# InfiniTensor/InfiniTensor

Hardware: AMD Instinct MI355X
Metric: bf16 MatMul 4096x4096x4096 throughput (GEMM TFLOP/s, % dense MFMA peak) (higher is better)
Workload: dtype bf16; 1 GPU; BASELINE configs[1]: one bf16 MatMul M=N=K=4096 per GPU, NN layout, fp32 accumulate, via infini_rocm_matmul; kernel_variant=heuristic, kernel_variant_launched=wave128, device=AMD Radeon Graphics, arch=gfx950:sramecc+:xnack-, compute_units=256, clock_mhz=2400, parallelism=1 independent replicas (column-sharded GEMM has no collective)

## Files before the change

infinitensor_amd/csrc/gemm128w.hip:

```cpp
#include "gemm256_common.h"
#include "diag.h"

namespace irocm {
namespace g128w {

using g256::mn_f;
using g256::sfor;

constexpr int kStage = 32768, kOper = 16384;
constexpr int kLds = 4 * kStage;
constexpr int kGroupM = 4;

struct WArgs {
    GemmArgs g;
    int total_tiles;
    int dbg;
    unsigned long long *stamps;
};
#ifdef IROCM_DIAG
constexpr bool kDiag = true;
#else
constexpr bool kDiag = false;
#endif
constexpr int kStamps = 8;

template <bool KMAJOR> struct Frags;
template <> struct Frags<true> {
    s16x8_t v[3][8];
    unsigned base[2];
    __device__ __forceinline__ void init(unsigned lds_oper, int half, int l15, int g4) {
        const int slot = (l15 & 1) | (((l15 >> 3) & 1) << 1) | (((l15 >> 1) & 3) << 2);
        base[0] = lds_oper + (unsigned)(half * 8192 + slot * 64 + ((g4 ^ (slot >> 2)) & 3) * 16);
        base[1] = base[0] + 2u * kStage;
    }
    template <int SET, int F, int STAGE, int DST = F> __device__ __forceinline__ void read0() {
        asm volatile("ds_read_b128 %0, %1 offset:%2" : "=v"(v[SET][DST]) : "v"(base[STAGE >> 1]), "i"(F * 1024 + (STAGE & 1) * kStage));
    }
    template <int SET, int F, int STAGE, int DST = F> __device__ __forceinline__ void read1() {}
    template <int SET, int F> __device__ __forceinline__ s16x8_t get() const { return v[SET][F]; }
};
template <> struct Frags<false> {
    s16x4_t lo[3][8], hi[3][8];
    unsigned addr[8];
    __device__ __forceinline__ void init(unsigned lds_oper, int half, int l15, int g4) {
        const int mnf = ((l15 >> 2) & 3) | ((g4 & 1) << 2);
        const unsigned mn_lane = (unsigned)((g4 * 8 + (l15 >> 2)) * 512 + (l15 & 1) * 8);
#pragma unroll
        for (int f = 0; f < 8; ++f) {
            const int c16 = ((l15 >> 1) & 1) | (((half * 8 + f) ^ mnf) << 1);
            addr[f] = lds_oper + mn_lane + (unsigned)c16 * 16u;
        }
    }
    template <int SET, int F, int STAGE, int DST = F> __device__ __forceinline__ void read0() {
        const unsigned a = STAGE >= 2 ? addr[F] + 2u * kStage : addr[F];
        asm volatile("ds_read_b64_tr_b16 %0, %1 offset:%2" : "=v"(lo[SET][DST]) : "v"(a), "i"((STAGE & 1) * kStage));
    }
    template <int SET, int F, int STAGE, int DST = F> __device__ __forceinline__ void read1() {
        const unsigned a = STAGE >= 2 ? addr[F] + 2u * kStage : addr[F];
        asm volatile("ds_read_b64_tr_b16 %0, %1 offset:%2" : "=v"(hi[SET][DST]) : "v"(a), "i"((STAGE & 1) * kStage + 2048));
    }
    template <int SET, int F> __device__ __forceinline__ s16x8_t get() const {
        return s16x8_t{lo[SET][F][0], lo[SET][F][1], lo[SET][F][2], lo[SET][F][3], hi[SET][F][0], hi[SET][F][1], hi[SET][F][2], hi[SET][F][3]};
    }
};

template <bool KMAJOR> __device__ __forceinline__ void piece_offs(unsigned (&off)[4], long ld, int w, int lane) {
#pragma unroll
    for (int i = 0; i < 4; ++i) {
        const int piece = w * 4 + i;
        if constexpr (KMAJOR) {
            const int slot = lane >> 2;
            const int r = piece * 16 + ((slot & 1) | (((slot >> 2) & 3) << 1) | (((slot >> 1) & 1) << 3));
            const int c_log = (lane & 3) ^ ((slot >> 2) & 3);
            off[i] = (unsigned)(((long)r * ld + c_log * 8) * 2);
        } else {
            const int kr = piece * 2 + (lane >> 5);
            const int c_log = (lane & 31) ^ (mn_f(kr) << 1);
            off[i] = (unsigned)(((long)kr * ld + c_log * 8) * 2);
        }
    }
}

struct PieceSel {
    int oper, idx, stage, imm;
};
template <bool AKM, bool BKM> constexpr int step_pieces(int S) { return (AKM ? ((S & 1) ? 8 : 0) : 4) + (BKM ? ((S & 1) ? 8 : 0) : 4); }
template <bool AKM, bool BKM> constexpr PieceSel piece_sel(int S, int q) {
    const int na = AKM ? ((S & 1) ? 8 : 0) : 4;
    const int oper = q < na ? 0 : 1, r = q < na ? q : q - na;
    const bool km = oper == 0 ? AKM : BKM;
    if (!km)
        return {oper, r, (S + 3) & 3, 0};
    return {oper, r >> 1, (r & 1) ? (S & 3) : ((S + 3) & 3), (r & 1) * 64};
}
constexpr int slot_piece(int n, int I, int slot) {
    if (n == 0)
        return -1;
    if (n <= 8) {
        const int stride = 8 / n;
        return (slot == 0 && I % stride == 0) ? I / stride : -1;
    }
    return slot == 0 ? I : (8 + I < n ? 8 + I : -1);
}

template <typename Tr> __device__ __forceinline__ unsigned cvt_pk_a(float lo, float hi) {
    unsigned r;
    if constexpr (Tr::kDType == INFINI_DT_BF16) asm volatile("v_cvt_pk_bf16_f32 %0, %1, %2" : "=v"(r) : "v"(lo), "v"(hi));
    else asm volatile("v_cvt_pk_f16_f32 %0, %1, %2" : "=v"(r) : "v"(lo), "v"(hi));
    return r;
}
#ifdef IROCM_W128_C_WB
#define W128_ST_MOD ""
#else
#define W128_ST_MOD " sc0 sc1"
#endif
struct EpiUnit {
    int kind, jp, t;
};
constexpr int kEpiUnits = 60;
constexpr EpiUnit epi_unit(int e) {
    const int kind[12] = {0, 0, 1, 0, 2, 1, 0, 2, 1, 2, 1, 2};
    const int jp[12] = {0, 1, 0, 2, 0, 1, 3, 1, 2, 2, 3, 3};
    const int size[12] = {12, 12, 2, 12, 1, 2, 12, 1, 2, 1, 2, 1};
    int s = 0;
    for (int i = 0; i < 12; ++i) {
        if (e < s + size[i])
            return {kind[i], jp[i], e - s};
        s += size[i];
    }
    return {-1, 0, 0};
}

template <typename Tr, bool FIRST> __device__ __forceinline__ void mfma_a(f32x4 &acc, s16x8_t x, s16x8_t y) {
    if constexpr (Tr::kDType == INFINI_DT_BF16) {
        if constexpr (FIRST) asm volatile("v_mfma_f32_16x16x32_bf16 %0, %1, %2, 0" : "=a"(acc) : "v"(x), "v"(y));
        else asm volatile("v_mfma_f32_16x16x32_bf16 %0, %1, %2, %0" : "+a"(acc) : "v"(x), "v"(y));
    } else {
        if constexpr (FIRST) asm volatile("v_mfma_f32_16x16x32_f16 %0, %1, %2, 0" : "=a"(acc) : "v"(x), "v"(y));
        else asm volatile("v_mfma_f32_16x16x32_f16 %0, %1, %2, %0" : "+a"(acc) : "v"(x), "v"(y));
    }
}

template <typename Tr, bool AKM, bool BKM>
__global__ __launch_bounds__(256, 1) void gemm128w_kernel(WArgs pw) {
    extern __shared__ __attribute__((aligned(1024))) char smem[];
    const GemmArgs &p = pw.g;
    unsigned long long tc0 = 0, tr0 = 0;
    if constexpr (kDiag) {
        tc0 = __builtin_amdgcn_s_memtime();
        tr0 = __builtin_amdgcn_s_memrealtime();
    }
    const int t = threadIdx.x, lane = t & 63, l15 = lane & 15, g4 = lane >> 4;
    int w;
    asm volatile("v_readfirstlane_b32 %0, %1" : "=s"(w) : "v"(t >> 6));
    const int wr = w >> 1, wc = w & 1;
    const unsigned lds0 = (unsigned)(unsigned long)IROCM_LDS_PTR(smem);
    unsigned lds0s;
    asm volatile("v_readfirstlane_b32 %0, %1" : "=s"(lds0s) : "v"(lds0));

    const long lda = AKM ? p.a_rs : p.a_cs, ldb = BKM ? p.b_cs : p.b_rs;
    unsigned a_kstep = (unsigned)(AKM ? 64 : 64 * lda), b_kstep = (unsigned)(BKM ? 64 : 64 * ldb);
    const long a_tile = AKM ? 512 * lda : 512, b_tile = BKM ? 512 * ldb : 512;
    unsigned a_off[4], b_off[4];
    piece_offs<AKM>(a_off, lda, w, lane);
    piece_offs<BKM>(b_off, ldb, w, lane);
    if (pw.dbg & 2) {
        a_kstep = b_kstep = 0;
#pragma unroll
        for (int i = 0; i < 4; ++i) a_off[i] = b_off[i] = (unsigned)lane * 16u;
    }
    const int ksteps = p.k >> 5, nkb = ksteps >> 2;
    const unsigned a_span = a_kstep * (unsigned)ksteps, b_span = b_kstep * (unsigned)ksteps;

    const unsigned grid = gridDim.x, wg = xcd_remap(blockIdx.x, grid);
    const unsigned per_batch = (unsigned)(p.tiles_m * p.tiles_n);
    auto decode = [&](unsigned tile, const char *&ab, const char *&bb, long &c_elem) {
        const unsigned ib = tile / per_batch, r = tile - ib * per_batch;
        const unsigned gspan = (unsigned)(kGroupM * p.tiles_n), grp = r / gspan, i = r - grp * gspan;
        const unsigned first_m = grp * kGroupM;
        const unsigned gsz = (unsigned)p.tiles_m - first_m < (unsigned)kGroupM ? (unsigned)p.tiles_m - first_m : (unsigned)kGroupM;
        const unsigned tn = i / gsz, tm = first_m + (i - tn * gsz);
        ab = (const char *)p.a + ((long)ib * p.a_bs) * 2 + (long)tm * a_tile;
        bb = (const char *)p.b + ((long)ib * p.b_bs) * 2 + (long)tn * b_tile;
        c_elem = (long)ib * p.c_bs + (long)tm * 256 * p.n + (long)tn * 256;
    };
    auto uniform = [](const char *q) {
        const unsigned long v = (unsigned long)q;
        const unsigned lo = __builtin_amdgcn_readfirstlane((unsigned)v), hi = __builtin_amdgcn_readfirstlane((unsigned)(v >> 32));
        return (const char *)(((unsigned long)hi << 32) | lo);
    };

    unsigned tile = wg;
    const char *pa, *pb;
    long c_elem;
    decode(tile, pa, pb, c_elem);
    pa = uniform(pa);
    pb = uniform(pb);

    unsigned m0w = lds0s + (unsigned)w * 4096u;
    auto load_piece = [&](auto operc, auto idxc, auto immc) __attribute__((always_inline)) {
        constexpr int OP = decltype(operc)::value, IDX = decltype(idxc)::value, IMM = decltype(immc)::value;
        const unsigned off = OP == 0 ? a_off[IDX] : b_off[IDX];
        const char *base = OP == 0 ? pa : pb;
        asm volatile("global_load_lds_dwordx4 %0, %1 offset:%2" ::"v"(off), "s"(base), "i"(IMM) : "memory");
    };
    auto set_m0 = [&m0w](auto stc, auto operc, auto idxc, auto immc) __attribute__((always_inline)) {
        constexpr int ST = decltype(stc)::value, OP = decltype(operc)::value, IDX = decltype(idxc)::value, IMM = decltype(immc)::value;
        const unsigned m0base = m0w;
        asm volatile("s_add_u32 m0, %0, %1" ::"s"(m0base), "i"(ST * kStage + OP * kOper + IDX * 1024 - IMM) : "memory", "scc");
    };
    auto pin = [&]() __attribute__((always_inline)) { asm volatile("" : "+s"(pa), "+s"(pb)); };
    auto request = [&](auto stc, auto operc) __attribute__((always_inline)) {
        constexpr int ST = decltype(stc)::value, OP = decltype(operc)::value;
        constexpr bool KM = OP == 0 ? AKM : BKM;
        sfor<4>([&](auto idxc) {
            set_m0(stc, operc, idxc, std::integral_constant<int, 0>{});
            asm volatile("s_nop 0" ::: "memory");
            load_piece(operc, idxc, std::integral_constant<int, 0>{});
            if constexpr (KM) {
                set_m0(std::integral_constant<int, ST + 1>{}, operc, idxc, std::integral_constant<int, 64>{});
                asm volatile("s_nop 0" ::: "memory");
                load_piece(operc, idxc, std::integral_constant<int, 64>{});
            }
        });
    };
    auto advance = [&](auto operc, unsigned by) __attribute__((always_inline)) {
#pragma unroll
        for (int i = 0; i < 4; ++i) {
            if constexpr (decltype(operc)::value == 0) a_off[i] += by;
            else b_off[i] += by;
        }
    };
    constexpr std::integral_constant<int, 0> kA{};
    constexpr std::integral_constant<int, 1> kB{};

    Frags<AKM> fa;
    Frags<BKM> fb;
    fa.init(lds0, wr, l15, g4);
    fb.init(lds0 + kOper, wc, l15, g4);
    f32x4 acc[8][8];

    constexpr int nKM = (AKM ? 1 : 0) + (BKM ? 1 : 0), nMN = 2 - nKM;
    pin();
    asm volatile("s_nop 4" ::: "memory");
    if constexpr (AKM) request(std::integral_constant<int, 0>{}, kA);
    if constexpr (BKM) request(std::integral_constant<int, 0>{}, kB);
    if constexpr (!AKM) request(std::integral_constant<int, 0>{}, kA);
    if constexpr (!BKM) request(std::integral_constant<int, 0>{}, kB);
    if constexpr (AKM) advance(kA, 128);
    else advance(kA, a_kstep);
    if constexpr (BKM) advance(kB, 128);
    else advance(kB, b_kstep);
    if constexpr (!AKM) request(std::integral_constant<int, 1>{}, kA);
    if constexpr (!BKM) request(std::integral_constant<int, 1>{}, kB);
    if constexpr (!AKM) advance(kA, a_kstep);
    if constexpr (!BKM) advance(kB, b_kstep);
    if constexpr (AKM) request(std::integral_constant<int, 2>{}, kA);
    if constexpr (BKM) request(std::integral_constant<int, 2>{}, kB);
    if constexpr (!AKM) request(std::integral_constant<int, 2>{}, kA);
    if constexpr (!BKM) request(std::integral_constant<int, 2>{}, kB);
    if constexpr (AKM) advance(kA, 128);
    else advance(kA, a_kstep);
    if constexpr (BKM) advance(kB, 128);
    else advance(kB, b_kstep);
    constexpr int kG1 = 4 * nMN, kG2 = 8 * nKM + 4 * nMN;
    asm volatile("s_waitcnt vmcnt(%0)" ::"n"(kG1 + kG2) : "memory");
    __builtin_amdgcn_s_barrier();
    sfor<8>([&](auto fc) {
        constexpr int F = decltype(fc)::value;
        fa.template read0<0, F, 0>();
        fa.template read1<0, F, 0>();
        fb.template read0<0, F, 0>();
        fb.template read1<0, F, 0>();
    });
    asm volatile("s_waitcnt vmcnt(%0) lgkmcnt(0)" ::"n"(kG2) : "memory");
    __builtin_amdgcn_s_barrier();

    const char *na = pa, *nb = pb;
    auto step = [&](auto sc, auto firstc, bool last_block) __attribute__((always_inline)) {
        constexpr int S = decltype(sc)::value;
        constexpr bool FIRST = decltype(firstc)::value;
        constexpr int CUR = S & 1, NXT = CUR ^ 1, RS = (S + 1) & 3, NP = step_pieces<AKM, BKM>(S);
        sfor<8>([&](auto ic) {
            constexpr int I = decltype(ic)::value;
            sfor<8>([&](auto jc) {
                constexpr int J = decltype(jc)::value;
                mfma_a<Tr, FIRST>(acc[I][J], fb.template get<CUR, J>(), fa.template get<CUR, I>());
                if constexpr (J == 0) fa.template read0<NXT, I, RS>();
                if constexpr (J == 1) fa.template read1<NXT, I, RS>();
                if constexpr (J == 2) fb.template read0<NXT, I, RS>();
                if constexpr (J == 3) fb.template read1<NXT, I, RS>();
                if constexpr (J >= 4) {
                    constexpr int Q = slot_piece(NP, I, (J - 4) >> 1);
                    if constexpr (Q >= 0) {
                        constexpr PieceSel ps = piece_sel<AKM, BKM>(S, Q);
                        if constexpr ((J & 1) == 0)
                            set_m0(std::integral_constant<int, ps.stage>{}, std::integral_constant<int, ps.oper>{}, std::integral_constant<int, ps.idx>{},
                                   std::integral_constant<int, ps.imm>{});
                        else
                            load_piece(std::integral_constant<int, ps.oper>{}, std::integral_constant<int, ps.idx>{}, std::integral_constant<int, ps.imm>{});
                    }
                }
            });
        });
        if (S == 0 && last_block) {
            pa = na;
            pb = nb;
            pin();
            advance(kA, AKM ? 0u - a_span : a_kstep - a_span);
            advance(kB, BKM ? 0u - b_span : b_kstep - b_span);
        } else {
            if constexpr (!AKM) advance(kA, a_kstep);
            else if constexpr (S & 1) advance(kA, 128);
            if constexpr (!BKM) advance(kB, b_kstep);
            else if constexpr (S & 1) advance(kB, 128);
        }
        asm volatile("s_waitcnt vmcnt(%0) lgkmcnt(0)" ::"n"(NP) : "memory");
        __builtin_amdgcn_s_barrier();
    };
    constexpr std::integral_constant<int, 0> k0{};
    constexpr std::integral_constant<int, 1> k1{};
    constexpr std::integral_constant<int, 2> k2{};
    constexpr std::integral_constant<int, 3> k3{};
    auto block = [&](auto firstc, bool last_block) __attribute__((always_inline)) {
        step(k0, firstc, last_block);
        step(k1, std::false_type{}, last_block);
        step(k2, std::false_type{}, last_block);
        step(k3, std::false_type{}, last_block);
    };
    unsigned long long tc_first = 0, tr_first = 0, tc_mfma = 0, tr_mfma = 0, tc_store = 0;
    if constexpr (kDiag) {
        tc_first = __builtin_amdgcn_s_memtime();
        tr_first = __builtin_amdgcn_s_memrealtime();
    }
    const unsigned total = (unsigned)pw.total_tiles;
    const long ldc2 = (long)p.n * 2;
    auto final_block = [&]() __attribute__((always_inline)) {
        const int ln = (int)__builtin_amdgcn_mbcnt_hi(~0u, __builtin_amdgcn_mbcnt_lo(~0u, 0u));
        const unsigned c_lane = (unsigned)(((long)(ln & 15) * p.n + ((ln >> 4) & 1) * 16 + (ln >> 5) * 8) * 2);
        char *cw = (char *)p.c + (c_elem + (long)wr * 128 * p.n + wc * 128) * 2;
        cw = (char *)uniform(cw);
        unsigned pu[8], pv[8];
        float t0 = 0.f, t1 = 0.f;
        sfor<8>([&](auto ic) {
            constexpr int I = decltype(ic)::value;
            constexpr int SA = (I & 1) * 2, SN = ((I + 1) & 1) * 2;
            char *cb = cw + (long)(I > 0 ? I - 1 : 0) * 16 * ldc2;
            asm volatile("" : "+s"(cb));
            if constexpr (I > 0) asm volatile("s_waitcnt lgkmcnt(0)" ::: "memory");
            sfor<24>([&](auto mc) {
                constexpr int M = decltype(mc)::value, KS = M >> 3, J = M & 7;
                if constexpr (I == 0 && M == 8) {
                    asm volatile("s_waitcnt vmcnt(0) lgkmcnt(0)" ::: "memory");
                    __builtin_amdgcn_s_barrier();
                }
                if constexpr (I == 0 && M == 16) asm volatile("s_waitcnt lgkmcnt(0)" ::: "memory");
                if constexpr (KS == 0) mfma_a<Tr, false>(acc[I][J], fb.template get<1, J>(), fa.template get<1, I>());
                if constexpr (KS == 1) mfma_a<Tr, false>(acc[I][J], fb.template get<0, J>(), fa.template get<0, SA>());
                if constexpr (KS == 2) mfma_a<Tr, false>(acc[I][J], fb.template get<2, J>(), fa.template get<0, SA + 1>());
                if constexpr (I == 0 && KS == 0) {
                    fb.template read0<0, J, 2>();
                    fb.template read1<0, J, 2>();
                    if constexpr (J == 0) {
                        fa.template read0<0, 0, 2, 0>();
                        fa.template read1<0, 0, 2, 0>();
                    }
                }
                if constexpr (I == 0 && KS == 1) {
                    fb.template read0<2, J, 3>();
                    fb.template read1<2, J, 3>();
                    if constexpr (J == 0) {
                        fa.template read0<0, 0, 3, 1>();
                        fa.template read1<0, 0, 3, 1>();
                    }
                }
                if constexpr (I < 7 && M == 16) {
                    fa.template read0<0, I + 1, 2, SN>();
                    fa.template read1<0, I + 1, 2, SN>();
                }
                if constexpr (I < 7 && M == 17) {
                    fa.template read0<0, I + 1, 3, SN + 1>();
                    fa.template read1<0, I + 1, 3, SN + 1>();
                }
                if constexpr (I > 0) {
                    constexpr int R = I - 1, E0 = M * kEpiUnits / 24, E1 = (M + 1) * kEpiUnits / 24;
                    sfor<E1 - E0>([&](auto uc) {
                        constexpr EpiUnit un = epi_unit(E0 + decltype(uc)::value);
                        if constexpr (un.kind == 0) {
                            constexpr int Q = 2 * un.jp + un.t / 6, H = (un.t % 6) / 3, RR = un.t % 3;
                            if constexpr (RR < 2) {
                                const float src = acc[R][Q][2 * H + RR];
                                float dst;
                                asm volatile("v_accvgpr_read_b32 %0, %1" : "=v"(dst) : "a"(src));
                                if constexpr (RR == 0) t0 = dst;
                                else t1 = dst;
                            } else if constexpr (un.t < 6) {
                                pu[2 * un.jp + H] = cvt_pk_a<Tr>(t0, t1);
                            } else {
                                pv[2 * un.jp + H] = cvt_pk_a<Tr>(t0, t1);
                            }
                        } else if constexpr (un.kind == 1) {
                            unsigned x = pu[2 * un.jp + un.t], y = pv[2 * un.jp + un.t];
                            asm volatile("v_permlane16_swap_b32 %0, %1" : "+v"(x), "+v"(y));
                            pu[2 * un.jp + un.t] = x;
                            pv[2 * un.jp + un.t] = y;
                        } else {
                            const u32x4_t d = u32x4_t{pu[2 * un.jp], pu[2 * un.jp + 1], pv[2 * un.jp], pv[2 * un.jp + 1]};
                            const unsigned cl = c_lane;
                            char *cbs = cb;
                            asm volatile("global_store_dwordx4 %0, %1, %2 offset:%3" W128_ST_MOD ::"v"(cl), "v"(d), "s"(cbs), "i"(un.jp * 64) : "memory");
                        }
                    });
                }
            });
        });
    };
    auto epilogue = [&](auto firstrowc) __attribute__((always_inline)) {
        constexpr int FIRSTROW = decltype(firstrowc)::value;
        if constexpr (kDiag) {
            tc_mfma = __builtin_amdgcn_s_memtime();
            tr_mfma = __builtin_amdgcn_s_memrealtime();
        }
        asm volatile("s_nop 15\n\ts_nop 15" ::: "memory");
        const int ln = (int)__builtin_amdgcn_mbcnt_hi(~0u, __builtin_amdgcn_mbcnt_lo(~0u, 0u));
        const unsigned c_lane = (unsigned)(((long)(ln & 15) * p.n + ((ln >> 4) & 1) * 16 + (ln >> 5) * 8) * 2);
        char *cw = (char *)p.c + (c_elem + (long)wr * 128 * p.n + wc * 128) * 2;
        cw = (char *)uniform(cw);
        if (!(pw.dbg & 1))
        sfor<8>([&](auto ic) {
            constexpr int I = decltype(ic)::value;
            if constexpr (I < FIRSTROW) return;
            char *cb = cw + (long)I * 16 * ldc2;
            asm volatile("s_nop 4" : "+s"(cb));
            unsigned u[8], v[8];
#pragma unroll
            for (int jp = 0; jp < 4; ++jp) {
                const f32x4 x = acc[I][2 * jp], y = acc[I][2 * jp + 1];
                u[2 * jp] = Tr::pack2(x[0], x[1]);
                u[2 * jp + 1] = Tr::pack2(x[2], x[3]);
                v[2 * jp] = Tr::pack2(y[0], y[1]);
                v[2 * jp + 1] = Tr::pack2(y[2], y[3]);
            }
            asm volatile("s_nop 1\n\t"
                         "v_permlane16_swap_b32 %0, %8\n\tv_permlane16_swap_b32 %1, %9\n\tv_permlane16_swap_b32 %2, %10\n\t"
                         "v_permlane16_swap_b32 %3, %11\n\tv_permlane16_swap_b32 %4, %12\n\tv_permlane16_swap_b32 %5, %13\n\t"
                         "v_permlane16_swap_b32 %6, %14\n\tv_permlane16_swap_b32 %7, %15"
                         : "+v"(u[0]), "+v"(u[1]), "+v"(u[2]), "+v"(u[3]), "+v"(u[4]), "+v"(u[5]), "+v"(u[6]), "+v"(u[7]), "+v"(v[0]), "+v"(v[1]),
                           "+v"(v[2]), "+v"(v[3]), "+v"(v[4]), "+v"(v[5]), "+v"(v[6]), "+v"(v[7]));
            const u32x4_t d0 = u32x4_t{u[0], u[1], v[0], v[1]}, d1 = u32x4_t{u[2], u[3], v[2], v[3]};
            const u32x4_t d2 = u32x4_t{u[4], u[5], v[4], v[5]}, d3 = u32x4_t{u[6], u[7], v[6], v[7]};
            const unsigned cl = c_lane;
            asm volatile("global_store_dwordx4 %0, %1, %5" W128_ST_MOD "\n\tglobal_store_dwordx4 %0, %2, %5 offset:64" W128_ST_MOD "\n\t"
                         "global_store_dwordx4 %0, %3, %5 offset:128" W128_ST_MOD "\n\tglobal_store_dwordx4 %0, %4, %5 offset:192" W128_ST_MOD "\n\ts_nop 1" ::"v"(cl),
                         "v"(d0), "v"(d1), "v"(d2), "v"(d3), "s"(cb)
                         : "memory");
        });
        if constexpr (kDiag) tc_store = __builtin_amdgcn_s_memtime();
    };
    for (; tile + grid < total; tile += grid) {
        {
            long dummy;
            decode(tile + grid, na, nb, dummy);
            na = uniform(na);
            nb = uniform(nb);
        }
        block(std::true_type{}, nkb == 1);
        for (int kb = 1; kb < nkb; ++kb) block(std::false_type{}, kb == nkb - 1);
        epilogue(k0);
        const char *ta, *tb;
        decode(tile + grid, ta, tb, c_elem);
    }
    if (nkb == 1) {
        step(k0, std::true_type{}, false);
        final_block();
        epilogue(std::integral_constant<int, 7>{});
    } else {
        block(std::true_type{}, false);
        for (int kb = 1; kb < nkb - 1; ++kb) block(std::false_type{}, false);
        step(k0, std::false_type{}, false);
        final_block();
        epilogue(std::integral_constant<int, 7>{});
    }
    asm volatile("s_waitcnt vmcnt(0)" ::: "memory");
    if constexpr (kDiag) {
        const bool lane0 = w == 0 && __builtin_amdgcn_mbcnt_hi(~0u, __builtin_amdgcn_mbcnt_lo(~0u, 0u)) == 0;
        if ((pw.dbg & 16) && lane0) {
            unsigned long long *d = pw.stamps + (size_t)blockIdx.x * kStamps;
            d[0] = tc0, d[1] = tc_first, d[2] = tc_mfma, d[3] = tc_store, d[4] = __builtin_amdgcn_s_memtime();
            d[5] = tr0, d[6] = tr_mfma, d[7] = __builtin_amdgcn_s_memrealtime();
        }
        if ((pw.dbg & 8) && blockIdx.x == 0 && lane0) {
            unsigned long long *d = (unsigned long long *)p.c;
            d[0] = __builtin_amdgcn_s_memtime() - tc_first;
            d[1] = __builtin_amdgcn_s_memrealtime() - tr_first;
        }
    }
}

template <typename Tr> static int launch_t(infiniRocmRuntime_t rt, GemmArgs p, bool akm, bool bkm) {
    WArgs w;
    p.tiles_m = p.m / 256;
    p.tiles_n = p.n / 256;
    w.g = p;
    w.total_tiles = p.tiles_m * p.tiles_n * p.batch;
    const char *dbg = diag_getenv("IROCM_W128_DBG");
    w.dbg = dbg ? atoi(dbg) : 0;
    w.stamps = nullptr;
    const unsigned grid = (unsigned)(w.total_tiles < rt->num_cu ? w.total_tiles : rt->num_cu);
    if (w.dbg & 16) {
        void *ws = nullptr;
        if (int st = infini_rocm_workspace(rt, (size_t)grid * kStamps * sizeof(unsigned long long), &ws))
            return st;
        w.stamps = (unsigned long long *)ws;
    }
    return with_layout(akm, bkm, [&](auto ak, auto bk) -> int {
        auto kern = gemm128w_kernel<Tr, decltype(ak)::value, decltype(bk)::value>;
        IROCM_LDS_ATTR(kern, kLds, rt);
        hipLaunchKernelGGL(kern, dim3(grid), dim3(256), kLds, rt->stream, w);
        IROCM_LAUNCH_CHECK("gemm128w");
        return INFINI_ROCM_OK;
    });
}

int launch_gemm128w(infiniRocmRuntime_t rt, int dtype, const GemmArgs &p, bool akm, bool bkm) {
    if (!wave128_supported(gemm_problem(p, dtype, akm, bkm)))
        IROCM_FAIL(INFINI_ROCM_UNSUPPORTED, "gemm128w: this problem is outside the four-wave kernel's contract (gemm_route.h)");
    return dtype == INFINI_DT_BF16 ? launch_t<Bf16Traits>(rt, p, akm, bkm) : launch_t<F16Traits>(rt, p, akm, bkm);
}

}
}
```

Before: 1550 TFLOP/s.

## Precompute tile-decode constants on host and use magic-number division in kernel

Moves per-launch derived values (strides in bytes, tile counts, k-steps, spans, XCD remap quotient/remainder) into a flattened kernel argument struct computed on the host. Tile decoding now uses precomputed magic multipliers instead of integer division, keeping scalar registers. Debug branches are compiled out unless diagnostics are enabled, and the acc registers are pinned before the epilogue. It also adds compile-time options for store cache modifiers, line-bound store layout and an alternate epilogue ordering, all off by default. The aim is to cut scalar setup work and register pressure in the prologue and between tiles, at the cost of 32-bit offset arithmetic that assumes strides fit in 32 bits.

```diff
diff --git a/infinitensor_amd/csrc/gemm128w.hip b/infinitensor_amd/csrc/gemm128w.hip
--- a/infinitensor_amd/csrc/gemm128w.hip
+++ b/infinitensor_amd/csrc/gemm128w.hip
@@ -11,9 +11,23 @@
 constexpr int kLds = 4 * kStage;
 constexpr int kGroupM = 4;
 
-struct WArgs {
-    GemmArgs g;
-    int total_tiles;
+struct alignas(64) WArgs {
+    const char *a, *b;
+    long a_bs2, b_bs2;
+    unsigned a_tile, b_tile;
+    unsigned a_ld2, b_ld2;
+    unsigned per_batch, per_batch_m;
+    unsigned gspan, gspan_m;
+    unsigned tiles_m;
+    unsigned tail_sz, tail_m;
+    unsigned grid, grid_q, grid_r;
+    unsigned total_tiles;
+    unsigned nkb;
+    unsigned a_kstep, b_kstep;
+    unsigned a_span, b_span;
+    char *c;
+    long c_bs2;
+    unsigned ldc2;
     int dbg;
     unsigned long long *stamps;
 };
@@ -22,7 +36,7 @@
 #else
 constexpr bool kDiag = false;
 #endif
-constexpr int kStamps = 8;
+constexpr int kStamps = 9;
 
 template <bool KMAJOR> struct Frags;
 template <> struct Frags<true> {
@@ -64,7 +78,7 @@
     }
 };
 
-template <bool KMAJOR> __device__ __forceinline__ void piece_offs(unsigned (&off)[4], long ld, int w, int lane) {
+template <bool KMAJOR> __device__ __forceinline__ void piece_offs(unsigned (&off)[4], unsigned ld2, int w, int lane) {
 #pragma unroll
     for (int i = 0; i < 4; ++i) {
         const int piece = w * 4 + i;
@@ -72,11 +86,11 @@
             const int slot = lane >> 2;
             const int r = piece * 16 + ((slot & 1) | (((slot >> 2) & 3) << 1) | (((slot >> 1) & 1) << 3));
             const int c_log = (lane & 3) ^ ((slot >> 2) & 3);
-            off[i] = (unsigned)(((long)r * ld + c_log * 8) * 2);
+            off[i] = (unsigned)r * ld2 + (unsigned)c_log * 16u;
         } else {
             const int kr = piece * 2 + (lane >> 5);
             const int c_log = (lane & 31) ^ (mn_f(kr) << 1);
-            off[i] = (unsigned)(((long)kr * ld + c_log * 8) * 2);
+            off[i] = (unsigned)kr * ld2 + (unsigned)c_log * 16u;
         }
     }
 }
@@ -109,19 +123,36 @@
     else asm volatile("v_cvt_pk_f16_f32 %0, %1, %2" : "=v"(r) : "v"(lo), "v"(hi));
     return r;
 }
-#ifdef IROCM_W128_C_WB
+#if defined(IROCM_W128_C_WB)
 #define W128_ST_MOD ""
+#elif defined(IROCM_W128_ST) && IROCM_W128_ST == 1
+#define W128_ST_MOD " sc1"
+#elif defined(IROCM_W128_ST) && IROCM_W128_ST == 2
+#define W128_ST_MOD " nt"
+#elif defined(IROCM_W128_ST) && IROCM_W128_ST == 3
+#define W128_ST_MOD " sc0"
 #else
 #define W128_ST_MOD " sc0 sc1"
+#endif
+#ifdef IROCM_W128_LINE_BOUND
+constexpr bool kLineBound = true;
+#else
+constexpr bool kLineBound = false;
 #endif
 struct EpiUnit {
     int kind, jp, t;
 };
 constexpr int kEpiUnits = 60;
 constexpr EpiUnit epi_unit(int e) {
+#ifdef IROCM_W128_EPI_PAIRED
+    const int kind[12] = {0, 0, 1, 0, 1, 0, 1, 2, 2, 1, 2, 2};
+    const int jp[12] = {0, 1, 0, 2, 1, 3, 2, 0, 1, 3, 2, 3};
+    const int size[12] = {12, 12, 2, 12, 2, 12, 2, 1, 1, 2, 1, 1};
+#else
     const int kind[12] = {0, 0, 1, 0, 2, 1, 0, 2, 1, 2, 1, 2};
     const int jp[12] = {0, 1, 0, 2, 0, 1, 3, 1, 2, 2, 3, 3};
     const int size[12] = {12, 12, 2, 12, 1, 2, 12, 1, 2, 1, 2, 1};
+#endif
     int s = 0;
     for (int i = 0; i < 12; ++i) {
         if (e < s + size[i])
@@ -129,6 +160,16 @@
         s += size[i];
     }
     return {-1, 0, 0};
+}
+
+__device__ __forceinline__ void udivmod_s(unsigned n, unsigned d, unsigned m, unsigned &q, unsigned &r) {
+    q = __umulhi(n, m);
+    r = n - q * d;
+    unsigned q1 = q + 1;
+    asm("" : "+s"(q1));
+    const bool fix = r >= d;
+    q = fix ? q1 : q;
+    r = fix ? r - d : r;
 }
 
 template <typename Tr, bool FIRST> __device__ __forceinline__ void mfma_a(f32x4 &acc, s16x8_t x, s16x8_t y) {
@@ -144,13 +185,12 @@
 template <typename Tr, bool AKM, bool BKM>
 __global__ __launch_bounds__(256, 1) void gemm128w_kernel(WArgs pw) {
     extern __shared__ __attribute__((aligned(1024))) char smem[];
-    const GemmArgs &p = pw.g;
     unsigned long long tc0 = 0, tr0 = 0;
     if constexpr (kDiag) {
         tc0 = __builtin_amdgcn_s_memtime();
         tr0 = __builtin_amdgcn_s_memrealtime();
     }
-    const int t = threadIdx.x, lane = t & 63, l15 = lane & 15, g4 = lane >> 4;
+    const int t = threadIdx.x, lane = t & 63;
     int w;
     asm volatile("v_readfirstlane_b32 %0, %1" : "=s"(w) : "v"(t >> 6));
     const int wr = w >> 1, wc = w & 1;
@@ -158,44 +198,45 @@
     unsigned lds0s;
     asm volatile("v_readfirstlane_b32 %0, %1" : "=s"(lds0s) : "v"(lds0));
 
-    const long lda = AKM ? p.a_rs : p.a_cs, ldb = BKM ? p.b_cs : p.b_rs;
-    unsigned a_kstep = (unsigned)(AKM ? 64 : 64 * lda), b_kstep = (unsigned)(BKM ? 64 : 64 * ldb);
-    const long a_tile = AKM ? 512 * lda : 512, b_tile = BKM ? 512 * ldb : 512;
+    unsigned a_kstep = pw.a_kstep, b_kstep = pw.b_kstep;
+    unsigned a_span = pw.a_span, b_span = pw.b_span;
     unsigned a_off[4], b_off[4];
-    piece_offs<AKM>(a_off, lda, w, lane);
-    piece_offs<BKM>(b_off, ldb, w, lane);
-    if (pw.dbg & 2) {
-        a_kstep = b_kstep = 0;
+    piece_offs<AKM>(a_off, pw.a_ld2, w, lane);
+    piece_offs<BKM>(b_off, pw.b_ld2, w, lane);
+    if constexpr (kDiag) {
+        if (pw.dbg & 2) {
+            a_kstep = b_kstep = a_span = b_span = 0;
 #pragma unroll
-        for (int i = 0; i < 4; ++i) a_off[i] = b_off[i] = (unsigned)lane * 16u;
-    }
-    const int ksteps = p.k >> 5, nkb = ksteps >> 2;
-    const unsigned a_span = a_kstep * (unsigned)ksteps, b_span = b_kstep * (unsigned)ksteps;
-
-    const unsigned grid = gridDim.x, wg = xcd_remap(blockIdx.x, grid);
-    const unsigned per_batch = (unsigned)(p.tiles_m * p.tiles_n);
-    auto decode = [&](unsigned tile, const char *&ab, const char *&bb, long &c_elem) {
-        const unsigned ib = tile / per_batch, r = tile - ib * per_batch;
-        const unsigned gspan = (unsigned)(kGroupM * p.tiles_n), grp = r / gspan, i = r - grp * gspan;
+            for (int i = 0; i < 4; ++i) a_off[i] = b_off[i] = (unsigned)lane * 16u;
+        }
+    }
+    const int nkb = (int)pw.nkb;
+
+    const unsigned grid = pw.grid;
+    const unsigned xcd = blockIdx.x % kNumXcd, wg = xcd * pw.grid_q + (xcd < pw.grid_r ? xcd : pw.grid_r) + blockIdx.x / kNumXcd;
+    struct TileAt {
+        unsigned ib, tm, tn;
+    };
+    auto decode = [&](unsigned tile, const char *&ab, const char *&bb) -> TileAt {
+        unsigned ib, r, grp, i, tn, rm;
+        udivmod_s(tile, pw.per_batch, pw.per_batch_m, ib, r);
+        udivmod_s(r, pw.gspan, pw.gspan_m, grp, i);
         const unsigned first_m = grp * kGroupM;
-        const unsigned gsz = (unsigned)p.tiles_m - first_m < (unsigned)kGroupM ? (unsigned)p.tiles_m - first_m : (unsigned)kGroupM;
-        const unsigned tn = i / gsz, tm = first_m + (i - tn * gsz);
-        ab = (const char *)p.a + ((long)ib * p.a_bs) * 2 + (long)tm * a_tile;
-        bb = (const char *)p.b + ((long)ib * p.b_bs) * 2 + (long)tn * b_tile;
-        c_elem = (long)ib * p.c_bs + (long)tm * 256 * p.n + (long)tn * 256;
-    };
-    auto uniform = [](const char *q) {
-        const unsigned long v = (unsigned long)q;
-        const unsigned lo = __builtin_amdgcn_readfirstlane((unsigned)v), hi = __builtin_amdgcn_readfirstlane((unsigned)(v >> 32));
-        return (const char *)(((unsigned long)hi << 32) | lo);
+        const bool full = first_m + kGroupM <= pw.tiles_m;
+        udivmod_s(i, full ? (unsigned)kGroupM : pw.tail_sz, full ? 0x40000000u : pw.tail_m, tn, rm);
+        const unsigned tm = first_m + rm;
+        ab = pw.a + (long)ib * pw.a_bs2 + (long)((unsigned long)tm * pw.a_tile);
+        bb = pw.b + (long)ib * pw.b_bs2 + (long)((unsigned long)tn * pw.b_tile);
+        return {ib, tm, tn};
+    };
+    auto c_corner = [&](const TileAt &at) {
+        const unsigned long rows = ((unsigned long)__umulhi(at.tm, pw.ldc2) << 32) | (unsigned long)(at.tm * pw.ldc2);
+        return (long)at.ib * pw.c_bs2 + (long)(rows << 8) + (long)at.tn * 512;
     };
 
     unsigned tile = wg;
     const char *pa, *pb;
-    long c_elem;
-    decode(tile, pa, pb, c_elem);
-    pa = uniform(pa);
-    pb = uniform(pb);
+    TileAt at = decode(tile, pa, pb);
 
     unsigned m0w = lds0s + (unsigned)w * 4096u;
     auto load_piece = [&](auto operc, auto idxc, auto immc) __attribute__((always_inline)) {
@@ -236,8 +277,6 @@
 
     Frags<AKM> fa;
     Frags<BKM> fb;
-    fa.init(lds0, wr, l15, g4);
-    fb.init(lds0 + kOper, wc, l15, g4);
     f32x4 acc[8][8];
 
     constexpr int nKM = (AKM ? 1 : 0) + (BKM ? 1 : 0), nMN = 2 - nKM;
@@ -247,6 +286,11 @@
     if constexpr (BKM) request(std::integral_constant<int, 0>{}, kB);
     if constexpr (!AKM) request(std::integral_constant<int, 0>{}, kA);
     if constexpr (!BKM) request(std::integral_constant<int, 0>{}, kB);
+    int lane_f = lane;
+    asm volatile("" : "+v"(lane_f), "+s"(at.ib), "+s"(at.tm), "+s"(at.tn));
+    fa.init(lds0, wr, lane_f & 15, lane_f >> 4);
+    fb.init(lds0 + kOper, wc, lane_f & 15, lane_f >> 4);
+    long c_byte = c_corner(at);
     if constexpr (AKM) advance(kA, 128);
     else advance(kA, a_kstep);
     if constexpr (BKM) advance(kB, 128);
@@ -328,18 +372,19 @@
         step(k2, std::false_type{}, last_block);
         step(k3, std::false_type{}, last_block);
     };
-    unsigned long long tc_first = 0, tr_first = 0, tc_mfma = 0, tr_mfma = 0, tc_store = 0;
+    unsigned long long tc_first = 0, tr_first = 0, tc_mfma = 0, tr_mfma = 0, tc_store = 0, tc_store0 = 0;
     if constexpr (kDiag) {
         tc_first = __builtin_amdgcn_s_memtime();
         tr_first = __builtin_amdgcn_s_memrealtime();
     }
-    const unsigned total = (unsigned)pw.total_tiles;
-    const long ldc2 = (long)p.n * 2;
+    const unsigned total = pw.total_tiles;
+    const long ldc2 = (long)pw.ldc2;
+    auto c_lane_of = [&](int ln) { return (unsigned)(ln & 15) * pw.ldc2 + (unsigned)(((ln >> 4) & 1) * 32 + (ln >> 5) * 16); };
+    auto c_wave = [&]() { return pw.c + c_byte + (long)((unsigned long)((unsigned)wr * pw.ldc2) << 7) + wc * 256; };
     auto final_block = [&]() __attribute__((always_inline)) {
         const int ln = (int)__builtin_amdgcn_mbcnt_hi(~0u, __builtin_amdgcn_mbcnt_lo(~0u, 0u));
-        const unsigned c_lane = (unsigned)(((long)(ln & 15) * p.n + ((ln >> 4) & 1) * 16 + (ln >> 5) * 8) * 2);
-        char *cw = (char *)p.c + (c_elem + (long)wr * 128 * p.n + wc * 128) * 2;
-        cw = (char *)uniform(cw);
+        const unsigned c_lane = kLineBound ? (unsigned)(ln >> 3) * pw.ldc2 + (unsigned)(ln & 7) * 16u : c_lane_of(ln);
+        char *cw = c_wave();
         unsigned pu[8], pv[8];
         float t0 = 0.f, t1 = 0.f;
         sfor<8>([&](auto ic) {
@@ -347,6 +392,8 @@
             constexpr int SA = (I & 1) * 2, SN = ((I + 1) & 1) * 2;
             char *cb = cw + (long)(I > 0 ? I - 1 : 0) * 16 * ldc2;
             asm volatile("" : "+s"(cb));
+            char *cb8 = cb + 8 * ldc2;
+            if constexpr (kLineBound) asm volatile("" : "+s"(cb8));
             if constexpr (I > 0) asm volatile("s_waitcnt lgkmcnt(0)" ::: "memory");
             sfor<24>([&](auto mc) {
                 constexpr int M = decltype(mc)::value, KS = M >> 3, J = M & 7;
@@ -407,8 +454,11 @@
                         } else {
                             const u32x4_t d = u32x4_t{pu[2 * un.jp], pu[2 * un.jp + 1], pv[2 * un.jp], pv[2 * un.jp + 1]};
                             const unsigned cl = c_lane;
-                            char *cbs = cb;
-                            asm volatile("global_store_dwordx4 %0, %1, %2 offset:%3" W128_ST_MOD ::"v"(cl), "v"(d), "s"(cbs), "i"(un.jp * 64) : "memory");
+                            char *cbs = kLineBound && un.jp >= 2 ? cb8 : cb;
+                            if constexpr (kDiag && R == 0 && un.jp == 0) tc_store0 = __builtin_amdgcn_s_memtime();
+                            asm volatile("global_store_dwordx4 %0, %1, %2 offset:%3" W128_ST_MOD ::"v"(cl), "v"(d), "s"(cbs),
+                                         "i"(kLineBound ? (un.jp & 1) * 128 : un.jp * 64)
+                                         : "memory");
                         }
                     });
                 }
@@ -422,11 +472,19 @@
             tr_mfma = __builtin_amdgcn_s_memrealtime();
         }
         asm volatile("s_nop 15\n\ts_nop 15" ::: "memory");
+        sfor<8>([&](auto ic) {
+            constexpr int I = decltype(ic)::value;
+            if constexpr (I >= FIRSTROW) {
+                f32x4(&r)[8] = acc[I];
+                asm volatile("" : "+a"(r[0]), "+a"(r[1]), "+a"(r[2]), "+a"(r[3]), "+a"(r[4]), "+a"(r[5]), "+a"(r[6]), "+a"(r[7]));
+            }
+        });
         const int ln = (int)__builtin_amdgcn_mbcnt_hi(~0u, __builtin_amdgcn_mbcnt_lo(~0u, 0u));
-        const unsigned c_lane = (unsigned)(((long)(ln & 15) * p.n + ((ln >> 4) & 1) * 16 + (ln >> 5) * 8) * 2);
-        char *cw = (char *)p.c + (c_elem + (long)wr * 128 * p.n + wc * 128) * 2;
-        cw = (char *)uniform(cw);
-        if (!(pw.dbg & 1))
+        const unsigned c_lane = c_lane_of(ln);
+        char *cw = c_wave();
+        bool stores = true;
+        if constexpr (kDiag) stores = !(pw.dbg & 1);
+        if (stores)
         sfor<8>([&](auto ic) {
             constexpr int I = decltype(ic)::value;
             if constexpr (I < FIRSTROW) return;
@@ -458,17 +516,12 @@
         if constexpr (kDiag) tc_store = __builtin_amdgcn_s_memtime();
     };
     for (; tile + grid < total; tile += grid) {
-        {
-            long dummy;
-            decode(tile + grid, na, nb, dummy);
-            na = uniform(na);
-            nb = uniform(nb);
-        }
+        decode(tile + grid, na, nb);
         block(std::true_type{}, nkb == 1);
         for (int kb = 1; kb < nkb; ++kb) block(std::false_type{}, kb == nkb - 1);
         epilogue(k0);
         const char *ta, *tb;
-        decode(tile + grid, ta, tb, c_elem);
+        c_byte = c_corner(decode(tile + grid, ta, tb));
     }
     if (nkb == 1) {
         step(k0, std::true_type{}, false);
@@ -488,25 +541,51 @@
             unsigned long long *d = pw.stamps + (size_t)blockIdx.x * kStamps;
             d[0] = tc0, d[1] = tc_first, d[2] = tc_mfma, d[3] = tc_store, d[4] = __builtin_amdgcn_s_memtime();
             d[5] = tr0, d[6] = tr_mfma, d[7] = __builtin_amdgcn_s_memrealtime();
+            d[8] = tc_store0;
         }
         if ((pw.dbg & 8) && blockIdx.x == 0 && lane0) {
-            unsigned long long *d = (unsigned long long *)p.c;
+            unsigned long long *d = (unsigned long long *)pw.c;
             d[0] = __builtin_amdgcn_s_memtime() - tc_first;
             d[1] = __builtin_amdgcn_s_memrealtime() - tr_first;
         }
     }
 }
 
-template <typename Tr> static int launch_t(infiniRocmRuntime_t rt, GemmArgs p, bool akm, bool bkm) {
-    WArgs w;
-    p.tiles_m = p.m / 256;
-    p.tiles_n = p.n / 256;
-    w.g = p;
-    w.total_tiles = p.tiles_m * p.tiles_n * p.batch;
+template <typename Tr> static int launch_t(infiniRocmRuntime_t rt, const GemmArgs &p, bool akm, bool bkm) {
+    WArgs w{};
+    const unsigned tiles_m = (unsigned)(p.m / 256), tiles_n = (unsigned)(p.n / 256), ksteps = (unsigned)(p.k / 32);
+    const long lda = akm ? p.a_rs : p.a_cs, ldb = bkm ? p.b_cs : p.b_rs;
+    w.a = (const char *)p.a;
+    w.b = (const char *)p.b;
+    w.a_bs2 = p.a_bs * 2;
+    w.b_bs2 = p.b_bs * 2;
+    w.a_tile = (unsigned)(akm ? 512 * lda : 512);
+    w.b_tile = (unsigned)(bkm ? 512 * ldb : 512);
+    w.a_ld2 = (unsigned)(2 * lda);
+    w.b_ld2 = (unsigned)(2 * ldb);
+    w.per_batch = tiles_m * tiles_n;
+    w.per_batch_m = udiv_magic(w.per_batch);
+    w.gspan = (unsigned)kGroupM * tiles_n;
+    w.gspan_m = udiv_magic(w.gspan);
+    w.tiles_m = tiles_m;
+    w.tail_sz = tiles_m % (unsigned)kGroupM;
+    w.tail_m = udiv_magic(w.tail_sz);
+    w.total_tiles = w.per_batch * (unsigned)p.batch;
+    w.grid = w.total_tiles < (unsigned)rt->num_cu ? w.total_tiles : (unsigned)rt->num_cu;
+    w.grid_q = w.grid / kNumXcd;
+    w.grid_r = w.grid % kNumXcd;
+    w.nkb = ksteps / 4;
+    w.a_kstep = (unsigned)(akm ? 64 : 64 * lda);
+    w.b_kstep = (unsigned)(bkm ? 64 : 64 * ldb);
+    w.a_span = w.a_kstep * ksteps;
+    w.b_span = w.b_kstep * ksteps;
+    w.c = (char *)p.c;
+    w.c_bs2 = p.c_bs * 2;
+    w.ldc2 = (unsigned)p.n * 2u;
     const char *dbg = diag_getenv("IROCM_W128_DBG");
     w.dbg = dbg ? atoi(dbg) : 0;
     w.stamps = nullptr;
-    const unsigned grid = (unsigned)(w.total_tiles < rt->num_cu ? w.total_tiles : rt->num_cu);
+    const unsigned grid = w.grid;
     if (w.dbg & 16) {
         void *ws = nullptr;
         if (int st = infini_rocm_workspace(rt, (size_t)grid * kStamps * sizeof(unsigned long long), &ws))
```

Result: no change. 1564 TFLOP/s (median of 6 runs) (+0.9%).

## Widen final-block k-window to four steps with extra prefetch in last tile

Applied to the files above, without the earlier changes.

For the last tile per workgroup, when K is at least 512, the final k-block is restructured so its drain window covers four k-steps instead of three. The last normal step issues extra global-to-LDS loads of the next k-step using separate base pointers, which lets the final block's MFMA and epilogue overlap more loads. It also adds empty asm register pins on LDS fragment addresses to split live ranges. The cost is more fragment registers (four sets instead of three) and a more complex schedule, which may raise register pressure.

```diff
diff --git a/infinitensor_amd/csrc/gemm128w.hip b/infinitensor_amd/csrc/gemm128w.hip
--- a/infinitensor_amd/csrc/gemm128w.hip
+++ b/infinitensor_amd/csrc/gemm128w.hip
@@ -10,6 +10,16 @@
 constexpr int kStage = 32768, kOper = 16384;
 constexpr int kLds = 4 * kStage;
 constexpr int kGroupM = 4;
+#ifndef IROCM_W128_WINDOW
+#define IROCM_W128_WINDOW 4
+#endif
+constexpr int kWin = IROCM_W128_WINDOW;
+static_assert(kWin == 3 || kWin == 4, "the final block's window is three or four k-steps");
+constexpr int kWinMinK = 512;
+static_assert(kWinMinK >= 384 && kWinMinK % 128 == 0, "the window's path is a first block, a special block and the final block: three blocks of four k-steps at least");
+constexpr int kSets = kWin > 3 ? kWin : 3;
+constexpr int win_stage(int R, int ws) { return (4 - R + ws) & 3; }
+constexpr int win_set(int R, int ws) { return ws == 0 ? (R & 1) : (ws - 1 < (R & 1) ? ws - 1 : ws); }
 
 struct WArgs {
     GemmArgs g;
@@ -26,13 +36,14 @@
 
 template <bool KMAJOR> struct Frags;
 template <> struct Frags<true> {
-    s16x8_t v[3][8];
+    s16x8_t v[kSets][8];
     unsigned base[2];
     __device__ __forceinline__ void init(unsigned lds_oper, int half, int l15, int g4) {
         const int slot = (l15 & 1) | (((l15 >> 3) & 1) << 1) | (((l15 >> 1) & 3) << 2);
         base[0] = lds_oper + (unsigned)(half * 8192 + slot * 64 + ((g4 ^ (slot >> 2)) & 3) * 16);
         base[1] = base[0] + 2u * kStage;
     }
+    __device__ __forceinline__ void split_ranges() { asm volatile("" : "+v"(base[0]), "+v"(base[1])); }
     template <int SET, int F, int STAGE, int DST = F> __device__ __forceinline__ void read0() {
         asm volatile("ds_read_b128 %0, %1 offset:%2" : "=v"(v[SET][DST]) : "v"(base[STAGE >> 1]), "i"(F * 1024 + (STAGE & 1) * kStage));
     }
@@ -40,7 +51,7 @@
     template <int SET, int F> __device__ __forceinline__ s16x8_t get() const { return v[SET][F]; }
 };
 template <> struct Frags<false> {
-    s16x4_t lo[3][8], hi[3][8];
+    s16x4_t lo[kSets][8], hi[kSets][8];
     unsigned addr[8];
     __device__ __forceinline__ void init(unsigned lds_oper, int half, int l15, int g4) {
         const int mnf = ((l15 >> 2) & 3) | ((g4 & 1) << 2);
@@ -50,6 +61,10 @@
             const int c16 = ((l15 >> 1) & 1) | (((half * 8 + f) ^ mnf) << 1);
             addr[f] = lds_oper + mn_lane + (unsigned)c16 * 16u;
         }
+    }
+    __device__ __forceinline__ void split_ranges() {
+#pragma unroll
+        for (int f = 0; f < 8; ++f) asm volatile("" : "+v"(addr[f]));
     }
     template <int SET, int F, int STAGE, int DST = F> __device__ __forceinline__ void read0() {
         const unsigned a = STAGE >= 2 ? addr[F] + 2u * kStage : addr[F];
@@ -93,6 +108,7 @@
         return {oper, r, (S + 3) & 3, 0};
     return {oper, r >> 1, (r & 1) ? (S & 3) : ((S + 3) & 3), (r & 1) * 64};
 }
+template <bool AKM, bool BKM> constexpr PieceSel extra_sel(int S, int e) { return {(!AKM && !BKM) ? e >> 2 : (AKM ? 1 : 0), e & 3, S & 3, 0}; }
 constexpr int slot_piece(int n, int I, int slot) {
     if (n == 0)
         return -1;
@@ -198,10 +214,12 @@
     pb = uniform(pb);
 
     unsigned m0w = lds0s + (unsigned)w * 4096u;
-    auto load_piece = [&](auto operc, auto idxc, auto immc) __attribute__((always_inline)) {
+    const char *pa1 = pa, *pb1 = pb;
+    auto load_piece = [&](auto operc, auto idxc, auto immc, auto xc) __attribute__((always_inline)) {
         constexpr int OP = decltype(operc)::value, IDX = decltype(idxc)::value, IMM = decltype(immc)::value;
+        constexpr bool X = decltype(xc)::value;
         const unsigned off = OP == 0 ? a_off[IDX] : b_off[IDX];
-        const char *base = OP == 0 ? pa : pb;
+        const char *base = X ? (OP == 0 ? pa1 : pb1) : (OP == 0 ? pa : pb);
         asm volatile("global_load_lds_dwordx4 %0, %1 offset:%2" ::"v"(off), "s"(base), "i"(IMM) : "memory");
     };
     auto set_m0 = [&m0w](auto stc, auto operc, auto idxc, auto immc) __attribute__((always_inline)) {
@@ -216,11 +234,11 @@
         sfor<4>([&](auto idxc) {
             set_m0(stc, operc, idxc, std::integral_constant<int, 0>{});
             asm volatile("s_nop 0" ::: "memory");
-            load_piece(operc, idxc, std::integral_constant<int, 0>{});
+            load_piece(operc, idxc, std::integral_constant<int, 0>{}, std::false_type{});
             if constexpr (KM) {
                 set_m0(std::integral_constant<int, ST + 1>{}, operc, idxc, std::integral_constant<int, 64>{});
                 asm volatile("s_nop 0" ::: "memory");
-                load_piece(operc, idxc, std::integral_constant<int, 64>{});
+                load_piece(operc, idxc, std::integral_constant<int, 64>{}, std::false_type{});
             }
         });
     };
@@ -277,10 +295,10 @@
     __builtin_amdgcn_s_barrier();
 
     const char *na = pa, *nb = pb;
-    auto step = [&](auto sc, auto firstc, bool last_block) __attribute__((always_inline)) {
+    auto step_x = [&](auto sc, auto firstc, bool last_block, auto extrac) __attribute__((always_inline)) {
         constexpr int S = decltype(sc)::value;
-        constexpr bool FIRST = decltype(firstc)::value;
-        constexpr int CUR = S & 1, NXT = CUR ^ 1, RS = (S + 1) & 3, NP = step_pieces<AKM, BKM>(S);
+        constexpr bool FIRST = decltype(firstc)::value, EXTRA = decltype(extrac)::value;
+        constexpr int CUR = S & 1, NXT = CUR ^ 1, RS = (S + 1) & 3, NPN = step_pieces<AKM, BKM>(S), NP = NPN + (EXTRA ? 4 * nMN : 0);
         sfor<8>([&](auto ic) {
             constexpr int I = decltype(ic)::value;
             sfor<8>([&](auto jc) {
@@ -293,17 +311,20 @@
                 if constexpr (J >= 4) {
                     constexpr int Q = slot_piece(NP, I, (J - 4) >> 1);
                     if constexpr (Q >= 0) {
-                        constexpr PieceSel ps = piece_sel<AKM, BKM>(S, Q);
+                        constexpr bool X = Q >= NPN;
+                        constexpr PieceSel ps = X ? extra_sel<AKM, BKM>(S, Q - NPN) : piece_sel<AKM, BKM>(S, Q);
                         if constexpr ((J & 1) == 0)
                             set_m0(std::integral_constant<int, ps.stage>{}, std::integral_constant<int, ps.oper>{}, std::integral_constant<int, ps.idx>{},
                                    std::integral_constant<int, ps.imm>{});
                         else
-                            load_piece(std::integral_constant<int, ps.oper>{}, std::integral_constant<int, ps.idx>{}, std::integral_constant<int, ps.imm>{});
+                            load_piece(std::integral_constant<int, ps.oper>{}, std::integral_constant<int, ps.idx>{}, std::integral_constant<int, ps.imm>{},
+                                       std::integral_constant<bool, X>{});
                     }
                 }
             });
         });
-        if (S == 0 && last_block) {
+        if constexpr (EXTRA) {
+        } else if (S == 0 && last_block) {
             pa = na;
             pb = nb;
             pin();
@@ -318,6 +339,7 @@
         asm volatile("s_waitcnt vmcnt(%0) lgkmcnt(0)" ::"n"(NP) : "memory");
         __builtin_amdgcn_s_barrier();
     };
+    auto step = [&](auto sc, auto firstc, bool last_block) __attribute__((always_inline)) { step_x(sc, firstc, last_block, std::false_type{}); };
     constexpr std::integral_constant<int, 0> k0{};
     constexpr std::integral_constant<int, 1> k1{};
     constexpr std::integral_constant<int, 2> k2{};
@@ -335,7 +357,8 @@
     }
     const unsigned total = (unsigned)pw.total_tiles;
     const long ldc2 = (long)p.n * 2;
-    auto final_block = [&]() __attribute__((always_inline)) {
+    auto final_block = [&](auto rc) __attribute__((always_inline)) {
+        constexpr int R = decltype(rc)::value, S0 = R & 1, AS = S0 ^ 1, NM = 8 * R;
         const int ln = (int)__builtin_amdgcn_mbcnt_hi(~0u, __builtin_amdgcn_mbcnt_lo(~0u, 0u));
         const unsigned c_lane = (unsigned)(((long)(ln & 15) * p.n + ((ln >> 4) & 1) * 16 + (ln >> 5) * 8) * 2);
         char *cw = (char *)p.c + (c_elem + (long)wr * 128 * p.n + wc * 128) * 2;
@@ -344,52 +367,40 @@
         float t0 = 0.f, t1 = 0.f;
         sfor<8>([&](auto ic) {
             constexpr int I = decltype(ic)::value;
-            constexpr int SA = (I & 1) * 2, SN = ((I + 1) & 1) * 2;
+            constexpr int SA = (I & 1) * (R - 1), SN = ((I + 1) & 1) * (R - 1);
             char *cb = cw + (long)(I > 0 ? I - 1 : 0) * 16 * ldc2;
             asm volatile("" : "+s"(cb));
             if constexpr (I > 0) asm volatile("s_waitcnt lgkmcnt(0)" ::: "memory");
-            sfor<24>([&](auto mc) {
-                constexpr int M = decltype(mc)::value, KS = M >> 3, J = M & 7;
+            sfor<NM>([&](auto mc) {
+                constexpr int M = decltype(mc)::value, WS = M >> 3, J = M & 7;
                 if constexpr (I == 0 && M == 8) {
                     asm volatile("s_waitcnt vmcnt(0) lgkmcnt(0)" ::: "memory");
                     __builtin_amdgcn_s_barrier();
                 }
-                if constexpr (I == 0 && M == 16) asm volatile("s_waitcnt lgkmcnt(0)" ::: "memory");
-                if constexpr (KS == 0) mfma_a<Tr, false>(acc[I][J], fb.template get<1, J>(), fa.template get<1, I>());
-                if constexpr (KS == 1) mfma_a<Tr, false>(acc[I][J], fb.template get<0, J>(), fa.template get<0, SA>());
-                if constexpr (KS == 2) mfma_a<Tr, false>(acc[I][J], fb.template get<2, J>(), fa.template get<0, SA + 1>());
-                if constexpr (I == 0 && KS == 0) {
-                    fb.template read0<0, J, 2>();
-                    fb.template read1<0, J, 2>();
+                if constexpr (I == 0 && WS >= 2 && J == 0) asm volatile("s_waitcnt lgkmcnt(0)" ::: "memory");
+                if constexpr (WS == 0) mfma_a<Tr, false>(acc[I][J], fb.template get<S0, J>(), fa.template get<S0, I>());
+                else mfma_a<Tr, false>(acc[I][J], fb.template get<win_set(R, WS), J>(), fa.template get<AS, SA + WS - 1>());
+                if constexpr (I == 0 && WS < R - 1) {
+                    constexpr int ST = win_stage(R, WS + 1), BS = win_set(R, WS + 1);
+                    fb.template read0<BS, J, ST>();
+                    fb.template read1<BS, J, ST>();
                     if constexpr (J == 0) {
-                        fa.template read0<0, 0, 2, 0>();
-                        fa.template read1<0, 0, 2, 0>();
+                        fa.template read0<AS, 0, ST, WS>();
+                        fa.template read1<AS, 0, ST, WS>();
                     }
                 }
-                if constexpr (I == 0 && KS == 1) {
-                    fb.template read0<2, J, 3>();
-                    fb.template read1<2, J, 3>();
-                    if constexpr (J == 0) {
-                        fa.template read0<0, 0, 3, 1>();
-                        fa.template read1<0, 0, 3, 1>();
-                    }
-                }
-                if constexpr (I < 7 && M == 16) {
-                    fa.template read0<0, I + 1, 2, SN>();
-                    fa.template read1<0, I + 1, 2, SN>();
-                }
-                if constexpr (I < 7 && M == 17) {
-                    fa.template read0<0, I + 1, 3, SN + 1>();
-                    fa.template read1<0, I + 1, 3, SN + 1>();
+                if constexpr (I < 7 && WS == R - 1 && J < R - 1) {
+                    fa.template read0<AS, I + 1, win_stage(R, J + 1), SN + J>();
+                    fa.template read1<AS, I + 1, win_stage(R, J + 1), SN + J>();
                 }
                 if constexpr (I > 0) {
-                    constexpr int R = I - 1, E0 = M * kEpiUnits / 24, E1 = (M + 1) * kEpiUnits / 24;
+                    constexpr int RT = I - 1, E0 = M * kEpiUnits / NM, E1 = (M + 1) * kEpiUnits / NM;
                     sfor<E1 - E0>([&](auto uc) {
                         constexpr EpiUnit un = epi_unit(E0 + decltype(uc)::value);
                         if constexpr (un.kind == 0) {
                             constexpr int Q = 2 * un.jp + un.t / 6, H = (un.t % 6) / 3, RR = un.t % 3;
                             if constexpr (RR < 2) {
-                                const float src = acc[R][Q][2 * H + RR];
+                                const float src = acc[RT][Q][2 * H + RR];
                                 float dst;
                                 asm volatile("v_accvgpr_read_b32 %0, %1" : "=v"(dst) : "a"(src));
                                 if constexpr (RR == 0) t0 = dst;
@@ -457,6 +468,10 @@
         });
         if constexpr (kDiag) tc_store = __builtin_amdgcn_s_memtime();
     };
+    auto split_ranges = [&]() __attribute__((always_inline)) {
+        fa.split_ranges();
+        fb.split_ranges();
+    };
     for (; tile + grid < total; tile += grid) {
         {
             long dummy;
@@ -464,37 +479,67 @@
             na = uniform(na);
             nb = uniform(nb);
         }
+        split_ranges();
         block(std::true_type{}, nkb == 1);
+        split_ranges();
         for (int kb = 1; kb < nkb; ++kb) block(std::false_type{}, kb == nkb - 1);
+        split_ranges();
         epilogue(k0);
         const char *ta, *tb;
         decode(tile + grid, ta, tb, c_elem);
     }
+    auto finish = [&]() __attribute__((always_inline)) {
+#ifdef IROCM_W128_NOWAIT
+        if constexpr (kDiag)
+#endif
+        asm volatile("s_waitcnt vmcnt(0)" ::: "memory");
+        if constexpr (kDiag) {
+            const bool lane0 = w == 0 && __builtin_amdgcn_mbcnt_hi(~0u, __builtin_amdgcn_mbcnt_lo(~0u, 0u)) == 0;
+            if ((pw.dbg & 16) && lane0) {
+                unsigned long long *d = pw.stamps + (size_t)blockIdx.x * kStamps;
+                d[0] = tc0, d[1] = tc_first, d[2] = tc_mfma, d[3] = tc_store, d[4] = __builtin_amdgcn_s_memtime();
+                d[5] = tr0, d[6] = tr_mfma, d[7] = __builtin_amdgcn_s_memrealtime();
+            }
+            if ((pw.dbg & 8) && blockIdx.x == 0 && lane0) {
+                unsigned long long *d = (unsigned long long *)p.c;
+                d[0] = __builtin_amdgcn_s_memtime() - tc_first;
+                d[1] = __builtin_amdgcn_s_memrealtime() - tr_first;
+            }
+        }
+    };
+    constexpr std::integral_constant<int, 3> w3{};
+    constexpr std::integral_constant<int, 7> row7{};
+    split_ranges();
+    if constexpr (kWin == 4) {
+        if (p.k >= kWinMinK) {
+            pa1 = pa + a_kstep;
+            pb1 = pb + b_kstep;
+            asm volatile("" : "+s"(pa1), "+s"(pb1));
+            split_ranges();
+            block(std::true_type{}, false);
+            for (int kb = 1; kb < nkb - 2; ++kb) block(std::false_type{}, false);
+            step(k0, std::false_type{}, false);
+            step(k1, std::false_type{}, false);
+            step(k2, std::false_type{}, false);
+            step_x(k3, std::false_type{}, false, std::true_type{});
+            final_block(std::integral_constant<int, kWin>{});
+            epilogue(row7);
+            finish();
+            __builtin_amdgcn_endpgm();
+        }
+    }
     if (nkb == 1) {
         step(k0, std::true_type{}, false);
-        final_block();
-        epilogue(std::integral_constant<int, 7>{});
+        final_block(w3);
+        epilogue(row7);
     } else {
         block(std::true_type{}, false);
         for (int kb = 1; kb < nkb - 1; ++kb) block(std::false_type{}, false);
         step(k0, std::false_type{}, false);
-        final_block();
-        epilogue(std::integral_constant<int, 7>{});
-    }
-    asm volatile("s_waitcnt vmcnt(0)" ::: "memory");
-    if constexpr (kDiag) {
-        const bool lane0 = w == 0 && __builtin_amdgcn_mbcnt_hi(~0u, __builtin_amdgcn_mbcnt_lo(~0u, 0u)) == 0;
-        if ((pw.dbg & 16) && lane0) {
-            unsigned long long *d = pw.stamps + (size_t)blockIdx.x * kStamps;
-            d[0] = tc0, d[1] = tc_first, d[2] = tc_mfma, d[3] = tc_store, d[4] = __builtin_amdgcn_s_memtime();
-            d[5] = tr0, d[6] = tr_mfma, d[7] = __builtin_amdgcn_s_memrealtime();
-        }
-        if ((pw.dbg & 8) && blockIdx.x == 0 && lane0) {
-            unsigned long long *d = (unsigned long long *)p.c;
-            d[0] = __builtin_amdgcn_s_memtime() - tc_first;
-            d[1] = __builtin_amdgcn_s_memrealtime() - tr_first;
-        }
-    }
+        final_block(w3);
+        epilogue(row7);
+    }
+    finish();
 }
 
 template <typename Tr> static int launch_t(infiniRocmRuntime_t rt, GemmArgs p, bool akm, bool bkm) {
```

Result: no change. 1463 TFLOP/s before, 1475 TFLOP/s after (median of 6 runs) (+0.8%).
